# kernrj/cuda-sdr

Measured on AMD Instinct MI355X. Metric: Msamples/sec through FIR→QuadAmDemod chain at 1/2/4/8 MI355X; % HBM roofline, higher is better.
Workload: dtype f32

## Files before the change

### cuda-sdr_amd/csrc/kernels/fir.hip

```cpp
#include "kcommon.h"
#include "fir_launch.h"

#include <gsdr/gsdr.h>
#include <gsdr/gsdr_amd.h>

#include <atomic>
#include <cmath>
#include <type_traits>
#include <utility>

namespace gsdr_amd {

enum InKind : int { kInF32 = 0, kInCF32 = 1, kInI8IQ = 2 };

constexpr int kR = 8;
constexpr int kRowBytes = 80;
constexpr int kThreads = 256;
constexpr int kWaves = kThreads / kWave;
constexpr int kWaveOutputs = kWave * kR;
constexpr int kFlushGroups = 8;

struct FirArgs {
  const void* in;
  const float* taps;
// ... 637 lines not shown

struct MixSpec {
  bool on = false;
  uint64_t phase0 = 0, step = 0;
};

template <int... Q>
void (*decFFTable(std::integer_sequence<int, Q...>, int qm))(FirArgs) {
  static void (*const kTable[])(FirArgs) = {firDecFFKernel<Q + 1>...};
  return kTable[qm - 1];
}
inline void (*decFFKernel(int qm))(FirArgs) { return decFFTable(std::make_integer_sequence<int, kDecMaxQ>{}, qm); }

template <int MODE, int INK, int EPI>
hipError_t launchFir(const void* in, const float* taps, size_t tapCount, size_t decimation, void* out,
                     size_t nOut, int32_t device, hipStream_t stream, MixSpec mix = MixSpec{}, float fmGain = 0.0f) {
  if (nOut == 0) return hipSuccess;
  if (in == nullptr || taps == nullptr || out == nullptr || tapCount == 0) return hipErrorInvalidValue;
  if (tapCount > 0x7fffffff || decimation > 0x7fffffff) return hipErrorInvalidValue;
  DevicePush push(device);
  if (!push.ok) return hipErrorInvalidDevice;

  if constexpr (MODE == kFirFC && (INK == kInI8IQ || INK == kInCF32) && EPI != kEpiPair && EPI != kEpiFm) {
    const bool smallCf = kFftSmallToMfma && INK == kInCF32 && !mix.on && decimation >= 2 &&
                         (uint64_t)nOut * decimation < kFftMinCf32Samples &&
                         (kernelPolicy() & (GSDR_POLICY_NO_MFMA | GSDR_POLICY_PREFER_FFT)) == 0 &&
                         firCfMfmaEligible(tapCount, decimation, in);
    if (!smallCf && (kernelPolicy() & (GSDR_POLICY_NO_FFT | GSDR_POLICY_NO_MFMA)) == 0 &&
        firFftEligible(tapCount, decimation, in, INK == kInI8IQ, mix.on))
      return launchFirFft(in, INK == kInI8IQ, taps, tapCount, decimation, out, nOut, EPI, stream,
                          FftMix{mix.on, mix.phase0, mix.step});
  }
  if constexpr (MODE == kFirCC && INK == kInCF32 && (EPI == kEpiComplex || EPI == kEpiAm)) {
    if (!mix.on && (kernelPolicy() & (GSDR_POLICY_NO_FFT | GSDR_POLICY_NO_MFMA)) == 0 &&
        firFftEligible(tapCount, decimation, in, false, false))
      return launchFirFft(in, false, taps, tapCount, decimation, out, nOut, EPI, stream, FftMix{}, true);
  }
  if constexpr (MODE == kFirFC && INK == kInI8IQ && EPI != kEpiPair && EPI != kEpiFm) if (!mix.on) {
    if ((kernelPolicy() & GSDR_POLICY_NO_MFMA) == 0 && firI8MfmaEligible(tapCount, decimation, in))
      return launchFirI8Mfma(static_cast<const int8_t*>(in), taps, tapCount, out, nOut, EPI, stream);
    if ((kernelPolicy() & GSDR_POLICY_NO_MFMA) == 0 && firI8DecMfmaEligible(tapCount, decimation, in))
      return launchFirI8DecMfma(static_cast<const int8_t*>(in), taps, tapCount, decimation, out, nOut, EPI, stream);
  }
  if constexpr (MODE == kFirFC && INK == kInCF32 && EPI != kEpiPair && EPI != kEpiFm) if (!mix.on) {
    if ((kernelPolicy() & GSDR_POLICY_NO_MFMA) == 0 && firCfMfmaEligible(tapCount, decimation, in))
      return launchFirCfMfma(static_cast<const float*>(in), taps, tapCount, decimation, out, nOut, EPI, stream);
  }

  const FirPlanShape s = planFirShape(tapCount, decimation);
  FirArgs a{};
  a.in = in;
// ... 256 lines not shown

hipError_t gsdrInt8MixFirFCAmDemod(size_t decimation, const float* taps, size_t tapCount, const int8_t* inputIq,
                                   double phase0, double radiansPerSample, float* output, size_t outputCount,
                                   int32_t device, hipStream_t stream) {
  return launchFir<kFirFC, kInI8IQ, kEpiAm>(inputIq, taps, tapCount, decimation, output, outputCount, device, stream,
                                            mixSpec(phase0, radiansPerSample));
}

hipError_t gsdrFirCCAmDemod(size_t decimation, const hipFloatComplex* taps, size_t tapCount,
                            const hipFloatComplex* input, float* output, size_t outputCount, int32_t device,
                            hipStream_t stream) {
  return launchFir<kFirCC, kInCF32, kEpiAm>(input, reinterpret_cast<const float*>(taps), tapCount, decimation,
                                            output, outputCount, device, stream);
}

}
```

### cuda-sdr_amd/csrc/kernels/fir_fft.hip

```cpp
#include "kcommon.h"
#include "fir_launch.h"

#include <gsdr/gsdr.h>
#include <gsdr/gsdr_amd.h>

#include <atomic>
#include <cmath>


namespace gsdr_amd {
namespace fftfir {

__device__ unsigned long long gDirectBlocks;

#ifndef GSDR_FFT_STAMPS
#define GSDR_FFT_STAMPS 0
#endif
#ifndef GSDR_FFT_EXP
#define GSDR_FFT_EXP 0
#endif
#if GSDR_FFT_STAMPS
constexpr int kStampWaves = 256 * 8;
__device__ unsigned long long gFftStamps[kStampWaves * 4];
#endif
// ... 11 lines not shown
  const float* taps;
  void* out;
  int64_t nOut;
  int64_t inBytes;
  int64_t nBlocks;
  int64_t inRows;
  int32_t T;
  int32_t Q;
  int32_t V;
  float inScale;
  float guardRatio;
  uint64_t mixPhase0;
  uint64_t mixStep;
  int32_t outAligned;
  int32_t complexTaps;
};

__device__ __forceinline__ f2 tapAt(const Args& a, int j) {
  return a.complexTaps ? reinterpret_cast<const f2*>(a.taps)[j] : f2{a.taps[j], 0.0f};
}

__device__ __forceinline__ f2 turnExp(uint64_t frac) {
  double sn, cs;
  sincospi((double)(int64_t)frac * 1.0842021724855044e-19, &sn, &cs);
  return f2{(float)cs, (float)sn};
}
__device__ __forceinline__ f2 turnExpF(uint64_t frac) {
  const int32_t hi = (int32_t)(frac >> 40) << 8 >> 8;
  float sh, ch;
  sincospif((float)hi * 1.1920928955078125e-7f, &sh, &ch);
// ... 254 lines not shown
template <int D>
constexpr int kRowUnits = D / 2 + ((GSDR_FFT_PADROWS && D == 4) ? 1 : 0);
template <int D>
__device__ __forceinline__ int rowSwizzle(int row) {
  return D == 8 ? (row >> 2) & 3 : 0;
}

template <int D>
constexpr int scratchComplex(int input) {
  return input == kCf32 ? (128 * kRowUnits<D> > 2 * kXch ? 128 * kRowUnits<D> : 2 * kXch)
                        : ((1024 * D + 16) / 8 > 2 * kXch ? (1024 * D + 16 + 7) / 8 : 2 * kXch);
}

constexpr int kMixT = 8 * 64;

template <int D, int IN, bool MIX = false>
constexpr size_t ldsBytes() {
  return (size_t)(D * 8 * 64 + kTw + kWaves * scratchComplex<D>(IN) + (MIX ? kMixT : 0)) * sizeof(f2);
}

template <int D, int IN, int NW = kWaves, bool MIX = false>
__device__ void buildTables(const Args& a, f2* twAll, const Lds& L, int w, int l, f2* mixT = nullptr) {
  if constexpr (MIX) {
    for (int n = threadIdx.x; n < kMixT; n += NW * kWave) {
      const int lane = (n >> 1) & 63, j = 2 * (n >> 7) + (n & 1);
      mixT[n] = turnExp((uint64_t)((lane + 64 * j) * D) * a.mixStep);
    }
  }
  for (int n = threadIdx.x; n < kTw; n += NW * kWave) {
    const int stage = n >> 9, kp = (n >> 7) & 3, lane = (n >> 1) & 63, r = 2 * kp + (n & 1) + 1;
    const int lo = lane & 7, hi = lane >> 3;
    int e;
    switch (stage) {
      case 0: e = lane * r; break;
// ... 286 lines not shown
    }
  }
}

#ifndef GSDR_FFT_XCD
#define GSDR_FFT_XCD 1
#endif
__device__ __forceinline__ int xcdGroup(int i, int n) {
  if (!GSDR_FFT_XCD || (n & 7) != 0) return i;
  return (i & 7) * (n >> 3) + (i >> 3);
}
#ifndef GSDR_FFT_XCD_D
#define GSDR_FFT_XCD_D 0
#endif

template <int D, int IN, int EPI, bool MIX = false>
__global__ void __launch_bounds__(kThreads) firFftKernel(Args a) {
  extern __shared__ __attribute__((aligned(16))) f2 lds[];
  const int w = __builtin_amdgcn_readfirstlane(threadIdx.x >> 6), l = threadIdx.x & 63;
  f2* twAll = lds + D * 8 * 64;
  f2* mixT = twAll + kTw + kWaves * scratchComplex<D>(IN);
  Lds L;
  L.g = reinterpret_cast<f4*>(lds);
  L.tw = reinterpret_cast<const f4*>(twAll) + l;
  L.scratch = twAll + kTw + w * scratchComplex<D>(IN);
  buildTables<D, IN, kWaves, MIX>(a, twAll, L, w, l, mixT);
#if GSDR_FFT_STAMPS
  const unsigned long long st0 = __builtin_amdgcn_s_memtime(), rt0 = __builtin_amdgcn_s_memrealtime();
#endif

  const int64_t stride = (int64_t)gridDim.x * kWaves;
  const int grp = GSDR_FFT_XCD_D ? xcdGroup((int)blockIdx.x, (int)gridDim.x) : (int)blockIdx.x;
  for (int64_t b = (int64_t)grp * kWaves + w; b < a.nBlocks; b += stride) {
    Rows<D, IN> R;
    loadRows<D>(a, b, R, L.scratch, l);
    f2 t[8];
    if constexpr (MIX) {
      loadMixT(t, reinterpret_cast<const f4*>(mixT), l);
      if constexpr (IN == kCf32) {
#pragma unroll
        for (int j = 0; j < 8; ++j)
#pragma unroll
          for (int p = 0; p < D; ++p) R.v[j][p] = cmul(R.v[j][p], t[j]);
      }
    }
    if (!(GSDR_FFT_EXP & 8) && blockNeedsDirect<D, IN>(a, R, b, l)) {
      if (l == 0) atomicAdd(&gDirectBlocks, 1ull);
      directBlock<D, IN, EPI, MIX>(a, b, l);
      continue;
    }
    __builtin_amdgcn_s_setprio(2);
    convolveBlock<D, IN, EPI, MIX>(a, R, b, L, l, t);
    __builtin_amdgcn_s_setprio(0);
  }
#if GSDR_FFT_STAMPS
  const unsigned long long st1 = __builtin_amdgcn_s_memtime(), rt1 = __builtin_amdgcn_s_memrealtime();
  const int slot = (int)blockIdx.x * kWaves + w;
  if (l == 0 && slot < kStampWaves) {
    unsigned long long* s = gFftStamps + 4 * slot;
    s[0] = st0;
    s[1] = rt0;
    s[2] = st1;
    s[3] = rt1;
  }
#endif
}

constexpr int kPfWaves = 4;

template <int D>
struct PrefetchCf {
  f4 u[8][D / 2];
};

template <int D>
__device__ __forceinline__ void issueBlockLoads(const Args& a, int64_t b, PrefetchCf<D>& P, int l) {
  const int64_t off = b < a.nBlocks ? b * (int64_t)a.V * D * 8 : 0;
  const auto rs = blockRsrc((const char*)a.in + off, b < a.nBlocks ? a.inBytes - off : 0);
#pragma unroll
  for (int j = 0; j < 8; ++j)
// ... 242 lines not shown
}

}

namespace {

std::atomic<float> gFftGuard{8.0f};

int cuCount() {
  int dev = 0, n = 0;
  if (hipGetDevice(&dev) != hipSuccess || hipDeviceGetAttribute(&n, hipDeviceAttributeMultiprocessorCount, dev) != hipSuccess || n <= 0)
    return 256;
  return n;
}

template <int D, int IN, int EPI, bool MIX>
hipError_t launchD(fftfir::Args a, hipStream_t stream) {
  using namespace fftfir;
  auto kernel = firFftKernel<D, IN, EPI, MIX>;
  const size_t lds = ldsBytes<D, IN, MIX>();
  const hipError_t e = hipFuncSetAttribute((const void*)kernel, hipFuncAttributeMaxDynamicSharedMemorySize, (int)lds);
  if (e != hipSuccess) return e;
  const int64_t maxGroups = cuCount();
  int64_t groups = (a.nBlocks + kWaves - 1) / kWaves;
  if (groups > maxGroups) groups = maxGroups;

  hipLaunchKernelGGL(kernel, dim3((unsigned)groups), dim3(kThreads), lds, stream, a);
  return hipGetLastError();
}

template <int EPI>
hipError_t launchD1(fftfir::Args a, hipStream_t stream) {
  using namespace fftfir;
  auto kernel = firFftD1PfKernel<EPI>;
  const size_t lds = (size_t)(8 * 8 * 64 + kTw + kPfWaves * scratchComplex<8>(kCf32) + kTwD1) * sizeof(f2);
  const hipError_t e = hipFuncSetAttribute((const void*)kernel, hipFuncAttributeMaxDynamicSharedMemorySize, (int)lds);
  if (e != hipSuccess) return e;
  const int64_t maxGroups = cuCount();
  int64_t groups = (a.nBlocks + kPfWaves - 1) / kPfWaves;
  if (groups > maxGroups) groups = maxGroups;
  hipLaunchKernelGGL(kernel, dim3((unsigned)groups), dim3(kPfWaves * kWave), lds, stream, a);
  return hipGetLastError();
}
// ... 25 lines not shown
    if (mixed) return false;
    const size_t Q = (tapCount + 7) / 8;
    return !int8Iq && tapCount >= 256 && Q <= (size_t)fftfir::kM - 64 && ((uintptr_t)in & 15) == 0;
  }
  if (!(D == 2 || D == 4 || D == 6 || D == 8 || D == 10)) return false;
  const size_t Q = (tapCount + D - 1) / D;
  if (tapCount < 256 || Q > (size_t)fftfir::kM - 63) return false;
  const uintptr_t p = (uintptr_t)in;
  if (int8Iq)
    return (p & 3) == 0 && (mixed || (kernelPolicy() & GSDR_POLICY_PREFER_FFT) != 0 ||
                            (!firI8MfmaEligible(tapCount, decimation, in) && !firI8DecMfmaEligible(tapCount, decimation, in)));
  return (p & 15) == 0;
}

hipError_t launchFirFft(const void* in, bool int8Iq, const float* taps, size_t tapCount, size_t decimation,
                        void* out, size_t nOut, int epi, hipStream_t stream, FftMix mix, bool complexTaps) {
  using namespace fftfir;
  if (nOut == 0) return hipSuccess;
  if (complexTaps && (int8Iq || mix.on)) return hipErrorInvalidValue;
  const size_t D = decimation < 1 ? 1 : decimation;
  if (D == 1) {
    if (int8Iq || mix.on) return hipErrorInvalidValue;
    Args a{};
    a.in = in;
    a.taps = taps;
    a.out = out;
    a.nOut = (int64_t)nOut;
    a.T = (int32_t)tapCount;
    a.Q = (int32_t)((tapCount + 7) / 8);
    a.V = kM - a.Q;
    a.inBytes = (int64_t)(nOut - 1 + tapCount) * 8;
// ... 7 lines not shown
  }
  Args a{};
  a.in = in;
  a.taps = taps;
  a.out = out;
  a.nOut = (int64_t)nOut;
  a.T = (int32_t)tapCount;
  a.Q = (int32_t)((tapCount + D - 1) / D);
  a.V = kM - a.Q + 1;
  a.inBytes = (int64_t)((nOut - 1) * D + tapCount) * (int8Iq ? 2 : 8);
  a.nBlocks = ((int64_t)nOut + a.V - 1) / a.V;
  a.inRows = (int64_t)(((nOut - 1) * D + tapCount) / D);
  a.inScale = int8Iq ? 1.0f / 127.0f : 1.0f;
  a.guardRatio = gFftGuard.load(std::memory_order_relaxed);
  a.complexTaps = complexTaps ? 1 : 0;
  const bool am = epi == kEpiAm;
  if (mix.on) {
    a.mixPhase0 = mix.phase0;
    a.mixStep = mix.step;
    if (int8Iq) return am ? launchFft<kI8, kAm, true>(a, D, stream) : launchFft<kI8, kComplex, true>(a, D, stream);
    return am ? launchFft<kCf32, kAm, true>(a, D, stream) : launchFft<kCf32, kComplex, true>(a, D, stream);
  }
  if (int8Iq) return am ? launchFft<kI8, kAm>(a, D, stream) : launchFft<kI8, kComplex>(a, D, stream);
  return am ? launchFft<kCf32, kAm>(a, D, stream) : launchFft<kCf32, kComplex>(a, D, stream);
}

}

extern "C" {
void gsdrAmdSetFftGuard(float ratio) { gsdr_amd::gFftGuard.store(ratio, std::memory_order_relaxed); }
float gsdrAmdGetFftGuard(void) { return gsdr_amd::gFftGuard.load(std::memory_order_relaxed); }

hipError_t gsdrAmdFftDirectBlocks(int32_t device, uint64_t* count, int reset) {
  int prev = 0;
  hipError_t e = hipGetDevice(&prev);
  if (e != hipSuccess) return e;
  if ((e = hipSetDevice(device)) != hipSuccess) return e;
  unsigned long long v = 0;
  e = hipDeviceSynchronize();
// ... 11 lines not shown
```

### cuda-sdr_amd/csrc/kernels/fir_launch.h

```cpp
#pragma once

#include <stddef.h>

namespace gsdr_amd {

enum FirMode : int { kFirFF = 0, kFirFC = 1, kFirCC = 2, kFirCF = 3 };
enum FirEpilogue : int { kEpiComplex = 0, kEpiPair = 1, kEpiAm = 2, kEpiFm = 3 };

struct FirPlanShape {
  size_t decimation;
  size_t deff;
  size_t gtot;
  size_t gmax;
  int waveOutputSlices;
  size_t regionRows;
  size_t ldsBytes;
  size_t tileOutputs;
};

FirPlanShape planFirShape(size_t tapCount, size_t decimation);

}

#include <hip/hip_runtime_api.h>
// ... 11 lines not shown

bool firI8DecMfmaEligible(size_t tapCount, size_t decimation, const void* in);
hipError_t launchFirI8DecMfma(const int8_t* iq, const float* taps, size_t tapCount, size_t decimation, void* out,
                              size_t nOut, int epi, hipStream_t stream);
hipError_t launchFirI8DecMfmaAudio(const int8_t* iq, const float* taps, size_t tapCount, size_t decimation,
                                   float* amOut, size_t nOut, const float* amHist, size_t amH, const float* aTaps,
                                   size_t aT, size_t aD, float* aOut, size_t aN, hipStream_t stream);

struct FftMix {
  bool on = false;
  uint64_t phase0 = 0, step = 0;
};
bool firFftEligible(size_t tapCount, size_t decimation, const void* in, bool int8Iq, bool mixed = false);
hipError_t launchFirFft(const void* in, bool int8Iq, const float* taps, size_t tapCount, size_t decimation,
                        void* out, size_t nOut, int epi, hipStream_t stream, FftMix mix = FftMix{},
                        bool complexTaps = false);

uint32_t kernelPolicy();

}
```

### cuda-sdr_amd/csrc/runtime/filters.cpp

```cpp
#include "filters.h"

#include <cstring>

#include <gsdr/conversion.h>
#include <gsdr/gsdr.h>
#include <gsdr/gsdr_amd.h>

#include <algorithm>
#include <cmath>

namespace gsdr_rt {

namespace {

Result<std::vector<ImmutableRef<IBufferCopier>>> deviceOutputCopiers(IFactories* f, ICudaCommandQueue* q) noexcept {
  try {
    Ref<IBufferCopier> d2d;
    UNWRAP_OR_FWD_RESULT(d2d, f->getCudaBufferCopierFactory()->createBufferCopier(q, hipMemcpyDeviceToDevice));
    std::vector<ImmutableRef<IBufferCopier>> v;
    v.emplace_back(d2d.get().get());
    return {.status = Status_Success, .value = std::move(v)};
  }
  IF_CATCH_RETURN_RESULT;
}
// ... 50 lines not shown
      mElementType(elementType),
      mAllocator(allocator),
      mH2D(h2d),
      mDecimation(std::max<size_t>(1, decimation)),
      mQueue(queue),
      mInElem(inputElementSize(elementType)),
      mOutElem((tapType == SampleType_Float && elementType == SampleType_Float) ? sizeof(float)
                                                                                : 2 * sizeof(float)) {}

Status Fir::setTaps(const float* taps, size_t tapCount) noexcept {
  GS_REQUIRE_OR_RET_STATUS(taps != nullptr || tapCount == 0, "taps must be non-null when tapCount > 0");
  const size_t bytes = tapCount * (mTapType == SampleType_FloatComplex ? 2 * sizeof(float) : sizeof(float));
  if (mTaps == nullptr || mTaps->capacity() < bytes) UNWRAP_OR_FWD_STATUS(mTaps, mAllocator->allocate(bytes));
  if (bytes > 0) FWD_IF_ERR(mH2D->copy(mTaps->data(), taps, bytes));
  mTapCount = tapCount;
  return Status_Success;
}

size_t Fir::availableInputs() const noexcept {
  if (!inputPortsInitialized()) return 0;
  Result<const IBuffer> in = getPortInputBuffer(0);
  if (in.status != Status_Success) return 0;
  return in.value->range()->used() / mInElem;
}

size_t Fir::availableOutputs() const noexcept {
  const size_t n = availableInputs();
  if (mTapCount == 0 || n < mTapCount) return 0;
  return (n - (mTapCount - 1)) / mDecimation;
}

size_t Fir::getOutputDataSize(size_t port) noexcept {
// ... 8 lines not shown

Status Fir::readOutput(IBuffer** portOutputBuffers, size_t portCount) noexcept {
  GS_REQUIRE_OR_RET_STATUS(portCount != 0 && portOutputBuffers != nullptr && portOutputBuffers[0] != nullptr,
                           "Must have one output port");
  IBuffer* out = portOutputBuffers[0];
  Ref<IBuffer> in;
  UNWRAP_OR_FWD_STATUS(in, getPortInputBuffer(0));
  const size_t n = std::min(availableOutputs(), out->range()->remaining() / mOutElem);
  if (n == 0) return Status_Success;

  const int32_t dev = mQueue->cudaDevice();
  hipStream_t s = mQueue->cudaStream();
  const void* x = in->readPtr();
  void* y = out->writePtr();
  hipError_t e;
  if (mElementType == SampleType_Int8Complex) {
    e = gsdrInt8FirFC(mDecimation, mTaps->as<float>(), mTapCount, static_cast<const int8_t*>(x),
                      static_cast<hipFloatComplex*>(y), n, dev, s);
  } else if (mTapType == SampleType_Float && mElementType == SampleType_Float) {
    e = gsdrFirFF(mDecimation, mTaps->as<float>(), mTapCount, static_cast<const float*>(x), static_cast<float*>(y), n,
                  dev, s);
  } else if (mTapType == SampleType_Float) {
    e = gsdrFirFC(mDecimation, mTaps->as<float>(), mTapCount, static_cast<const hipFloatComplex*>(x),
                  static_cast<hipFloatComplex*>(y), n, dev, s);
  } else if (mElementType == SampleType_FloatComplex) {
    e = gsdrFirCC(mDecimation, mTaps->as<hipFloatComplex>(), mTapCount, static_cast<const hipFloatComplex*>(x),
                  static_cast<hipFloatComplex*>(y), n, dev, s);
  } else {
    e = gsdrFirCF(mDecimation, mTaps->as<hipFloatComplex>(), mTapCount, static_cast<const float*>(x),
                  static_cast<hipFloatComplex*>(y), n, dev, s);
  }
  SAFE_HIP_OR_RET_STATUS(e);
  FWD_IF_ERR(out->range()->increaseEndOffset(n * mOutElem));
  return consumeInputBytesAndMoveUsedToStart(0, n * mDecimation * mInElem);
}

Status Fir::readOutputAm(IBuffer* out) noexcept {
  GS_REQUIRE_OR_RET_STATUS(out != nullptr && canFuseAm(), "Fir::readOutputAm needs real taps and an output");
  Ref<IBuffer> in;
  UNWRAP_OR_FWD_STATUS(in, getPortInputBuffer(0));
  const size_t n = std::min(availableOutputs(), out->range()->remaining() / sizeof(float));
  if (n == 0) return Status_Success;
  const int32_t dev = mQueue->cudaDevice();
  hipStream_t s = mQueue->cudaStream();
  hipError_t e;
  if (mElementType == SampleType_Int8Complex)
    e = gsdrInt8FirFCAmDemod(mDecimation, mTaps->as<float>(), mTapCount, in->readPtr<int8_t>(), out->writePtr<float>(),
                             n, dev, s);
  else
    e = gsdrFirFCAmDemod(mDecimation, mTaps->as<float>(), mTapCount, in->readPtr<hipFloatComplex>(),
                         out->writePtr<float>(), n, dev, s);
  SAFE_HIP_OR_RET_STATUS(e);
  FWD_IF_ERR(out->range()->increaseEndOffset(n * sizeof(float)));
  return consumeInputBytesAndMoveUsedToStart(0, n * mDecimation * mInElem);
}

Result<Filter> QuadAmDemod::create(ICudaCommandQueue* queue, IFactories* factories) noexcept {
  NON_NULL_PARAM_OR_RET(queue);
  Ref<IRelocatableResizableBufferFactory> windows;
  Ref<IMemSet> memSet;
  UNWRAP_OR_FWD_RESULT(windows, factories->createRelocatableCudaBufferFactory(queue, 32, false));
// ... 392 lines not shown
```

### cuda-sdr_amd/csrc/runtime/filters.h

```cpp
#pragma once

#include "waiter.h"

#include <gpusdrpipeline/Factories.h>
#include <gpusdrpipeline/abi/base_filters.h>
#include <gpusdrpipeline/abi/errors.h>

#include "graph_state.h"

namespace gsdr_rt {

constexpr size_t kDevicePreferredBytes = size_t{256} << 20;

size_t inputElementSize(SampleType t) noexcept;

class Fir final : public BaseFilter, public IGraphStepState {
 public:
  hipStream_t graphStream() const noexcept final { return mQueue->cudaStream(); }
  bool graphState(uint64_t& h) const noexcept final {
    foldWindowState(h);
    h = (h ^ reinterpret_cast<uintptr_t>(mTaps.get() ? mTaps->data() : nullptr)) * 0x100000001B3ull + mTapCount;
    return true;
  }
  bool saveStepState(GraphNodeState& out) const noexcept final { return saveSinkWindows(*this, out); }
  Status restoreStepState(const GraphNodeState& in) noexcept final { return restoreSinkWindows(*this, in); }
  static Result<Filter> create(SampleType tapType, SampleType elementType, size_t decimation, const float* taps,
                               size_t tapCount, ICudaCommandQueue* queue, IFactories* factories) noexcept;

  size_t getOutputDataSize(size_t port) noexcept final;
  size_t getOutputSizeAlignment(size_t port) noexcept final;
  Status readOutput(IBuffer** portOutputBuffers, size_t numPorts) noexcept final;
  size_t preferredInputBufferSize(size_t port) noexcept final { return kDevicePreferredBytes; }

  size_t decimation() const noexcept { return mDecimation; }
  size_t tapCount() const noexcept { return mTapCount; }

// ... 8 lines not shown
 private:
  Fir(SampleType tapType, SampleType elementType, size_t decimation, ICudaCommandQueue* queue, IAllocator* allocator,
      IBufferCopier* h2d, IRelocatableResizableBufferFactory* windows, IBufferSliceFactory* slices, IMemSet* memSet,
      std::vector<ImmutableRef<IBufferCopier>>&& outputCopiers) noexcept;
  Status setTaps(const float* taps, size_t tapCount) noexcept;
  size_t availableInputs() const noexcept;
  size_t availableOutputs() const noexcept;

  const SampleType mTapType;
  const SampleType mElementType;
  ConstRef<IAllocator> mAllocator;
  ConstRef<IBufferCopier> mH2D;
  const size_t mDecimation;
  Ref<IMemory> mTaps;
  size_t mTapCount = 0;
  ConstRef<ICudaCommandQueue> mQueue;
  const size_t mInElem;
  const size_t mOutElem;

  REF_COUNTED(Fir);
};

class QuadAmDemod final : public BaseFilter, public IGraphStepState {
 public:
  hipStream_t graphStream() const noexcept final { return mQueue->cudaStream(); }
  bool graphState(uint64_t& h) const noexcept final {
    foldWindowState(h);
    return true;
  }
  bool saveStepState(GraphNodeState& out) const noexcept final { return saveSinkWindows(*this, out); }
  Status restoreStepState(const GraphNodeState& in) noexcept final { return restoreSinkWindows(*this, in); }
  static Result<Filter> create(ICudaCommandQueue* queue, IFactories* factories) noexcept;
  size_t getOutputDataSize(size_t port) noexcept final;
  size_t getOutputSizeAlignment(size_t port) noexcept final;
  Status readOutput(IBuffer** portOutputBuffers, size_t numPorts) noexcept final;
// ... 175 lines not shown
```

### cuda-sdr_amd/gpusdr/ops.py

```python
from __future__ import annotations

import ctypes

import torch

from ._native import HipError, check, lib


def _stream(t: torch.Tensor):
    return torch.cuda.current_stream(t.device).cuda_stream


def _dev(t: torch.Tensor) -> int:
    return t.device.index if t.device.index is not None else torch.cuda.current_device()


def _require(t: torch.Tensor, dtype, name: str):
    if not t.is_cuda:
        raise ValueError(f"{name} must be a device tensor")
    if t.dtype != dtype:
        raise ValueError(f"{name} must be {dtype}, got {t.dtype}")
    if not t.is_contiguous():
        raise ValueError(f"{name} must be contiguous")

# ... 83 lines not shown
    if out.numel() < num_outputs:
        raise ValueError("out too small")
    fn = getattr(lib(), _FIR_ENTRY[key])
    args = (d, taps.data_ptr(), T, x.data_ptr(), out.data_ptr(), int(num_outputs), _dev(x), _stream(x))
    name = fn.__name__
    keep = (taps, x, out)

    def launch():
        if num_outputs > 0:
            code = fn(*args)
            if code != 0:
                raise HipError(f"{name} failed with hipError_t {code} ({len(keep)} bound tensors)")
    return launch


def fir_am_i8_carry(taps: torch.Tensor, iq: torch.Tensor, decimation: int, num_outputs: int,
                    out: torch.Tensor, carry: torch.Tensor) -> torch.Tensor:
    _require(taps, torch.float32, "taps")
    _require(iq, torch.int8, "iq")
    _require(out, torch.float32, "out")
    _require(carry, torch.int8, "carry")
    d = max(1, int(decimation))
    T = taps.numel()
    if num_outputs > 0 and (num_outputs - 1) * d + T > iq.numel() // 2:
        raise ValueError("input too short for the requested outputs")
    if out.numel() < num_outputs or carry.numel() < 2 * max(0, T - d):
        raise ValueError("out or carry too small")
    check(lib().gsdrInt8FirFCAmDemodCarry(d, taps.data_ptr(), T, iq.data_ptr(), out.data_ptr(), num_outputs,
                                          carry.data_ptr(), _dev(iq), _stream(iq)), "gsdrInt8FirFCAmDemodCarry")
    return out
# ... 112 lines not shown
def synth_wideband_cf32(seed: int, f1: float, f2: float, first: int, n: int,
                        out: torch.Tensor | None = None, device="cuda") -> torch.Tensor:
    if out is None:
        out = torch.empty(n, dtype=torch.complex64, device=device)
    check(lib().gsdrSynthWidebandCf32(seed, f1, f2, first, out.data_ptr(), n, _dev(out), _stream(out)),
          "gsdrSynthWidebandCf32")
    return out


POLICY_NO_MFMA = 1
POLICY_CF_BF16 = 2
POLICY_NO_WS = 4
POLICY_NO_FFT = 8
POLICY_PREFER_FFT = 16
POLICY_I8_WS8 = 64


def kernel_policy() -> int:
    L = lib()
    L.gsdrAmdGetKernelPolicy.restype = ctypes.c_uint32
    return int(L.gsdrAmdGetKernelPolicy())


def set_kernel_policy(flags: int) -> int:
    L = lib()
    L.gsdrAmdGetKernelPolicy.restype = ctypes.c_uint32
    L.gsdrAmdSetKernelPolicy.argtypes = [ctypes.c_uint32]
    prev = L.gsdrAmdGetKernelPolicy()
    L.gsdrAmdSetKernelPolicy(flags)
    return prev
# ... 77 lines not shown
```

### include/gsdr/gsdr_amd.h

```cpp
#ifndef GSDR_GSDR_AMD_H
#define GSDR_GSDR_AMD_H

#include <gsdr/gsdr.h>

#ifdef __cplusplus
extern "C" {
#endif

GSDR_API hipError_t gsdrInt8FirFC(size_t decimation, const float* taps, size_t tapCount, const int8_t* inputIq,
                                  hipFloatComplex* output, size_t outputCount, int32_t device, hipStream_t stream);
GSDR_API hipError_t gsdrInt8FirFCAmDemod(size_t decimation, const float* taps, size_t tapCount,
                                         const int8_t* inputIq, float* output, size_t outputCount, int32_t device,
                                         hipStream_t stream);
GSDR_API hipError_t gsdrFirFCAmDemod(size_t decimation, const float* taps, size_t tapCount,
                                     const hipFloatComplex* input, float* output, size_t outputCount, int32_t device,
                                     hipStream_t stream);
GSDR_API hipError_t gsdrFirCCAmDemod(size_t decimation, const hipFloatComplex* taps, size_t tapCount,
                                     const hipFloatComplex* input, float* output, size_t outputCount, int32_t device,
                                     hipStream_t stream);

GSDR_API hipError_t gsdrInt8FirFCAmDemodFirFF(size_t decimation, const float* taps, size_t tapCount,
                                              const int8_t* inputIq, size_t rfCount, float* amWindow,
                                              size_t amHistory, int storeAm, size_t audioDecimation,
                                              const float* audioTaps, size_t audioTapCount, float* audioOut,
// ... 22 lines not shown
                                        hipStream_t stream);
GSDR_API hipError_t gsdrInt8MixFirFCFmDemod(size_t decimation, const float* taps, size_t tapCount,
                                            const int8_t* inputIq, double phase0, double radiansPerSample, float gain,
                                            float* output, size_t outputCount, int32_t device, hipStream_t stream);
GSDR_API hipError_t gsdrFmDemod(size_t rfSampleRate, float tunedFrequency, float channelFrequency,
                                float channelFmDeviation, size_t rfLowPassDecimation, size_t firstSampleOffset,
                                const float* taps, size_t tapCount, const hipFloatComplex* input, float* output,
                                size_t outputCount, int32_t device, hipStream_t stream);

#define GSDR_POLICY_NO_MFMA 1u
#define GSDR_POLICY_CF_BF16 2u
#define GSDR_POLICY_NO_WS 4u
#define GSDR_POLICY_NO_FFT 8u
#define GSDR_POLICY_PREFER_FFT 16u
#define GSDR_POLICY_I8_WS8 64u
GSDR_API void gsdrAmdSetKernelPolicy(uint32_t flags);
GSDR_API const char* gsdrAmdFirKernelClass(int int8Iq, size_t tapCount, size_t decimation, const void* input);
GSDR_API uint32_t gsdrAmdGetKernelPolicy(void);
GSDR_API void gsdrAmdSetFftGuard(float ratio);
GSDR_API float gsdrAmdGetFftGuard(void);
GSDR_API hipError_t gsdrAmdFftDirectBlocks(int32_t device, uint64_t* count, int reset);
GSDR_API void gsdrAmdSetWsSpinLimit(int32_t microseconds);
GSDR_API int32_t gsdrAmdGetWsSpinLimit(void);
GSDR_API hipError_t gsdrAmdWsAborts(int32_t device, uint64_t* count, int reset);
GSDR_API uint32_t gsdrAmdWsTakeAborts(int32_t device);
GSDR_API uint32_t gsdrAmdWsAbortsPending(int32_t device);
GSDR_API const char* gsdrAmdBuildId(void);
GSDR_API const char* gsdrAmdBuildCompiler(void);
GSDR_API hipError_t gsdrAmdHbmProbe(const void* input, void* output, size_t bytes, int32_t mode, int32_t device,
                                    hipStream_t stream);
GSDR_API hipError_t gsdrAmdPoisonLds(uint32_t pattern, int32_t device, hipStream_t stream);
GSDR_API hipError_t gsdrAmdCopyKernel(void* dst, const void* src, size_t bytes, hipStream_t stream);

GSDR_API hipError_t gsdrSynthIqInt8(uint64_t seed, double sampleRate, double amToneHz, double carrierHz,
                                    uint64_t firstSample, int8_t* outputIq, size_t numSamples, int32_t device,
// ... 62 lines not shown
```

Baseline: 545,100.

## Add FIR plan with precomputed FFT tables and narrower FFT blocks for small grids

```diff
diff --git a/cuda-sdr_amd/csrc/kernels/fir.hip b/cuda-sdr_amd/csrc/kernels/fir.hip
--- a/cuda-sdr_amd/csrc/kernels/fir.hip
+++ b/cuda-sdr_amd/csrc/kernels/fir.hip
@@ -675,7 +675,8 @@
 
 template <int MODE, int INK, int EPI>
 hipError_t launchFir(const void* in, const float* taps, size_t tapCount, size_t decimation, void* out,
-                     size_t nOut, int32_t device, hipStream_t stream, MixSpec mix = MixSpec{}, float fmGain = 0.0f) {
+                     size_t nOut, int32_t device, hipStream_t stream, MixSpec mix = MixSpec{}, float fmGain = 0.0f,
+                     const void* fftTables = nullptr) {
   if (nOut == 0) return hipSuccess;
   if (in == nullptr || taps == nullptr || out == nullptr || tapCount == 0) return hipErrorInvalidValue;
   if (tapCount > 0x7fffffff || decimation > 0x7fffffff) return hipErrorInvalidValue;
@@ -690,12 +691,12 @@
     if (!smallCf && (kernelPolicy() & (GSDR_POLICY_NO_FFT | GSDR_POLICY_NO_MFMA)) == 0 &&
         firFftEligible(tapCount, decimation, in, INK == kInI8IQ, mix.on))
       return launchFirFft(in, INK == kInI8IQ, taps, tapCount, decimation, out, nOut, EPI, stream,
-                          FftMix{mix.on, mix.phase0, mix.step});
+                          FftMix{mix.on, mix.phase0, mix.step}, false, fftTables);
   }
   if constexpr (MODE == kFirCC && INK == kInCF32 && (EPI == kEpiComplex || EPI == kEpiAm)) {
     if (!mix.on && (kernelPolicy() & (GSDR_POLICY_NO_FFT | GSDR_POLICY_NO_MFMA)) == 0 &&
         firFftEligible(tapCount, decimation, in, false, false))
-      return launchFirFft(in, false, taps, tapCount, decimation, out, nOut, EPI, stream, FftMix{}, true);
+      return launchFirFft(in, false, taps, tapCount, decimation, out, nOut, EPI, stream, FftMix{}, true, fftTables);
   }
   if constexpr (MODE == kFirFC && INK == kInI8IQ && EPI != kEpiPair && EPI != kEpiFm) if (!mix.on) {
     if ((kernelPolicy() & GSDR_POLICY_NO_MFMA) == 0 && firI8MfmaEligible(tapCount, decimation, in))
@@ -982,4 +983,49 @@
                                             output, outputCount, device, stream);
 }
 
-}
+hipError_t gsdrAmdFirPlanCreate(int32_t device, hipStream_t stream, const void* taps, size_t tapCount,
+                                size_t decimation, int32_t int8Iq, int32_t complexTaps, gsdrAmdFirPlan* planOut) {
+  if (planOut == nullptr) return hipErrorInvalidValue;
+  *planOut = nullptr;
+  DevicePush push(device);
+  if (!push.ok) return hipErrorInvalidDevice;
+  FirFftPlan* p = nullptr;
+  const hipError_t e = firFftPlanCreate(device, stream, static_cast<const float*>(taps), tapCount, decimation,
+                                        int8Iq != 0, complexTaps != 0, &p);
+  if (e == hipSuccess) *planOut = reinterpret_cast<gsdrAmdFirPlan>(p);
+  return e;
+}
+
+void gsdrAmdFirPlanDestroy(gsdrAmdFirPlan plan) {
+  FirFftPlan* p = reinterpret_cast<FirFftPlan*>(plan);
+  if (p == nullptr) return;
+  DevicePush push(p->device);
+  firFftPlanDestroy(p);
+}
+
+const void* gsdrAmdFirPlanTables(gsdrAmdFirPlan plan) {
+  return plan != nullptr ? reinterpret_cast<const FirFftPlan*>(plan)->tables : nullptr;
+}
+
+hipError_t gsdrAmdFirPlanLaunch(gsdrAmdFirPlan plan, int32_t amDemod, const void* input, void* output,
+                                size_t outputCount, hipStream_t stream) {
+  const FirFftPlan* p = reinterpret_cast<const FirFftPlan*>(plan);
+  if (p == nullptr) return hipErrorInvalidValue;
+  const size_t D = p->decimation, T = p->tapCount;
+  if (p->int8Iq)
+    return amDemod ? launchFir<kFirFC, kInI8IQ, kEpiAm>(input, p->taps, T, D, output, outputCount, p->device, stream,
+                                                        MixSpec{}, 0.0f, p->tables)
+                   : launchFir<kFirFC, kInI8IQ, kEpiComplex>(input, p->taps, T, D, output, outputCount, p->device,
+                                                             stream, MixSpec{}, 0.0f, p->tables);
+  if (p->complexTaps)
+    return amDemod ? launchFir<kFirCC, kInCF32, kEpiAm>(input, p->taps, T, D, output, outputCount, p->device, stream,
+                                                        MixSpec{}, 0.0f, p->tables)
+                   : launchFir<kFirCC, kInCF32, kEpiComplex>(input, p->taps, T, D, output, outputCount, p->device,
+                                                             stream, MixSpec{}, 0.0f, p->tables);
+  return amDemod ? launchFir<kFirFC, kInCF32, kEpiAm>(input, p->taps, T, D, output, outputCount, p->device, stream,
+                                                      MixSpec{}, 0.0f, p->tables)
+                 : launchFir<kFirFC, kInCF32, kEpiComplex>(input, p->taps, T, D, output, outputCount, p->device,
+                                                           stream, MixSpec{}, 0.0f, p->tables);
+}
+
+}
diff --git a/cuda-sdr_amd/csrc/kernels/fir_fft.hip b/cuda-sdr_amd/csrc/kernels/fir_fft.hip
--- a/cuda-sdr_amd/csrc/kernels/fir_fft.hip
+++ b/cuda-sdr_amd/csrc/kernels/fir_fft.hip
@@ -6,6 +6,7 @@
 
 #include <atomic>
 #include <cmath>
+#include <new>
 
 
 namespace gsdr_amd {
@@ -49,6 +50,7 @@
   uint64_t mixStep;
   int32_t outAligned;
   int32_t complexTaps;
+  const void* tables;
 };
 
 __device__ __forceinline__ f2 tapAt(const Args& a, int j) {
@@ -333,10 +335,12 @@
 
 constexpr int kMixT = 8 * 64;
 
-template <int D, int IN, bool MIX = false>
+template <int D, int IN, bool MIX = false, int NW = kWaves>
 constexpr size_t ldsBytes() {
-  return (size_t)(D * 8 * 64 + kTw + kWaves * scratchComplex<D>(IN) + (MIX ? kMixT : 0)) * sizeof(f2);
-}
+  return (size_t)(D * 8 * 64 + kTw + NW * scratchComplex<D>(IN) + (MIX ? kMixT : 0)) * sizeof(f2);
+}
+template <int D>
+constexpr int kTableUnits = (D * 8 * 64 + kTw) / 2;
 
 template <int D, int IN, int NW = kWaves, bool MIX = false>
 __device__ void buildTables(const Args& a, f2* twAll, const Lds& L, int w, int l, f2* mixT = nullptr) {
@@ -653,24 +657,31 @@
 #define GSDR_FFT_XCD_D 0
 #endif
 
-template <int D, int IN, int EPI, bool MIX = false>
-__global__ void __launch_bounds__(kThreads) firFftKernel(Args a) {
+template <int D, int IN, int EPI, bool MIX = false, int NW = kWaves>
+__global__ void __launch_bounds__(NW * kWave) firFftKernel(Args a) {
   extern __shared__ __attribute__((aligned(16))) f2 lds[];
   const int w = __builtin_amdgcn_readfirstlane(threadIdx.x >> 6), l = threadIdx.x & 63;
   f2* twAll = lds + D * 8 * 64;
-  f2* mixT = twAll + kTw + kWaves * scratchComplex<D>(IN);
+  f2* mixT = twAll + kTw + NW * scratchComplex<D>(IN);
   Lds L;
   L.g = reinterpret_cast<f4*>(lds);
   L.tw = reinterpret_cast<const f4*>(twAll) + l;
   L.scratch = twAll + kTw + w * scratchComplex<D>(IN);
-  buildTables<D, IN, kWaves, MIX>(a, twAll, L, w, l, mixT);
+  if (!MIX && a.tables != nullptr) {
+    const f4* src = reinterpret_cast<const f4*>(a.tables);
+    f4* dst = reinterpret_cast<f4*>(lds);
+    for (int n = threadIdx.x; n < kTableUnits<D>; n += NW * kWave) dst[n] = src[n];
+    __syncthreads();
+  } else {
+    buildTables<D, IN, NW, MIX>(a, twAll, L, w, l, mixT);
+  }
 #if GSDR_FFT_STAMPS
   const unsigned long long st0 = __builtin_amdgcn_s_memtime(), rt0 = __builtin_amdgcn_s_memrealtime();
 #endif
 
-  const int64_t stride = (int64_t)gridDim.x * kWaves;
+  const int64_t stride = (int64_t)gridDim.x * NW;
   const int grp = GSDR_FFT_XCD_D ? xcdGroup((int)blockIdx.x, (int)gridDim.x) : (int)blockIdx.x;
-  for (int64_t b = (int64_t)grp * kWaves + w; b < a.nBlocks; b += stride) {
+  for (int64_t b = (int64_t)grp * NW + w; b < a.nBlocks; b += stride) {
     Rows<D, IN> R;
     loadRows<D>(a, b, R, L.scratch, l);
     f2 t[8];
@@ -694,7 +705,7 @@
   }
 #if GSDR_FFT_STAMPS
   const unsigned long long st1 = __builtin_amdgcn_s_memtime(), rt1 = __builtin_amdgcn_s_memrealtime();
-  const int slot = (int)blockIdx.x * kWaves + w;
+  const int slot = (int)blockIdx.x * NW + w;
   if (l == 0 && slot < kStampWaves) {
     unsigned long long* s = gFftStamps + 4 * slot;
     s[0] = st0;
@@ -703,6 +714,20 @@
     s[3] = rt1;
   }
 #endif
+}
+
+template <int D>
+__global__ void __launch_bounds__(kThreads) firFftTablesKernel(Args a, f4* image) {
+  extern __shared__ __attribute__((aligned(16))) f2 lds[];
+  const int w = __builtin_amdgcn_readfirstlane(threadIdx.x >> 6), l = threadIdx.x & 63;
+  f2* twAll = lds + D * 8 * 64;
+  Lds L;
+  L.g = reinterpret_cast<f4*>(lds);
+  L.tw = reinterpret_cast<const f4*>(twAll) + l;
+  L.scratch = twAll + kTw + w * scratchComplex<D>(kCf32);
+  buildTables<D, kCf32, kWaves, false>(a, twAll, L, w, l);
+  const f4* src = reinterpret_cast<const f4*>(lds);
+  for (int n = threadIdx.x; n < kTableUnits<D>; n += kThreads) image[n] = src[n];
 }
 
 constexpr int kPfWaves = 4;
@@ -975,19 +1000,31 @@
   return n;
 }
 
+template <int D, int IN, int EPI, bool MIX, int NW>
+hipError_t launchNW(fftfir::Args a, int64_t maxGroups, hipStream_t stream) {
+  using namespace fftfir;
+  auto kernel = firFftKernel<D, IN, EPI, MIX, NW>;
+  const size_t lds = ldsBytes<D, IN, MIX, NW>();
+  const hipError_t e = hipFuncSetAttribute((const void*)kernel, hipFuncAttributeMaxDynamicSharedMemorySize, (int)lds);
+  if (e != hipSuccess) return e;
+  int64_t groups = (a.nBlocks + NW - 1) / NW;
+  if (groups > maxGroups) groups = maxGroups;
+
+  hipLaunchKernelGGL(kernel, dim3((unsigned)groups), dim3(NW * kWave), lds, stream, a);
+  return hipGetLastError();
+}
+
 template <int D, int IN, int EPI, bool MIX>
 hipError_t launchD(fftfir::Args a, hipStream_t stream) {
   using namespace fftfir;
-  auto kernel = firFftKernel<D, IN, EPI, MIX>;
-  const size_t lds = ldsBytes<D, IN, MIX>();
-  const hipError_t e = hipFuncSetAttribute((const void*)kernel, hipFuncAttributeMaxDynamicSharedMemorySize, (int)lds);
-  if (e != hipSuccess) return e;
-  const int64_t maxGroups = cuCount();
-  int64_t groups = (a.nBlocks + kWaves - 1) / kWaves;
-  if (groups > maxGroups) groups = maxGroups;
-
-  hipLaunchKernelGGL(kernel, dim3((unsigned)groups), dim3(kThreads), lds, stream, a);
-  return hipGetLastError();
+  const int64_t cus = cuCount();
+  if constexpr (!MIX) {
+    if (a.nBlocks < cus * kWaves && (kernelPolicy() & GSDR_POLICY_FFT_GRID8) == 0) {
+      if (a.nBlocks <= cus * 2) return launchNW<D, IN, EPI, MIX, 2>(a, cus, stream);
+      if (a.nBlocks <= cus * 4) return launchNW<D, IN, EPI, MIX, 4>(a, cus, stream);
+    }
+  }
+  return launchNW<D, IN, EPI, MIX, kWaves>(a, cus, stream);
 }
 
 template <int EPI>
@@ -1043,7 +1080,8 @@
 }
 
 hipError_t launchFirFft(const void* in, bool int8Iq, const float* taps, size_t tapCount, size_t decimation,
-                        void* out, size_t nOut, int epi, hipStream_t stream, FftMix mix, bool complexTaps) {
+                        void* out, size_t nOut, int epi, hipStream_t stream, FftMix mix, bool complexTaps,
+                        const void* tables) {
   using namespace fftfir;
   if (nOut == 0) return hipSuccess;
   if (complexTaps && (int8Iq || mix.on)) return hipErrorInvalidValue;
@@ -1081,6 +1119,7 @@
   a.inScale = int8Iq ? 1.0f / 127.0f : 1.0f;
   a.guardRatio = gFftGuard.load(std::memory_order_relaxed);
   a.complexTaps = complexTaps ? 1 : 0;
+  a.tables = mix.on ? nullptr : tables;
   const bool am = epi == kEpiAm;
   if (mix.on) {
     a.mixPhase0 = mix.phase0;
@@ -1090,6 +1129,72 @@
   }
   if (int8Iq) return am ? launchFft<kI8, kAm>(a, D, stream) : launchFft<kI8, kComplex>(a, D, stream);
   return am ? launchFft<kCf32, kAm>(a, D, stream) : launchFft<kCf32, kComplex>(a, D, stream);
+}
+
+namespace {
+template <int D>
+hipError_t launchTables(fftfir::Args a, void* image, hipStream_t stream) {
+  using namespace fftfir;
+  auto kernel = firFftTablesKernel<D>;
+  const size_t lds = ldsBytes<D, kCf32>();
+  const hipError_t e = hipFuncSetAttribute((const void*)kernel, hipFuncAttributeMaxDynamicSharedMemorySize, (int)lds);
+  if (e != hipSuccess) return e;
+  hipLaunchKernelGGL(kernel, dim3(1), dim3(kThreads), lds, stream, a, reinterpret_cast<f4*>(image));
+  return hipGetLastError();
+}
+}
+
+hipError_t firFftPlanCreate(int32_t device, hipStream_t stream, const float* taps, size_t tapCount, size_t decimation,
+                            bool int8Iq, bool complexTaps, FirFftPlan** planOut) {
+  using namespace fftfir;
+  if (planOut == nullptr) return hipErrorInvalidValue;
+  *planOut = nullptr;
+  if (taps == nullptr || tapCount == 0 || tapCount > 0x7fffffff || decimation > 0x7fffffff || (int8Iq && complexTaps))
+    return hipErrorInvalidValue;
+  const size_t D = decimation < 1 ? 1 : decimation;
+  FirFftPlan* p = new (std::nothrow) FirFftPlan;
+  if (p == nullptr) return hipErrorOutOfMemory;
+  p->device = device;
+  p->tapCount = tapCount;
+  p->decimation = D;
+  p->int8Iq = int8Iq;
+  p->complexTaps = complexTaps;
+  const size_t tapBytes = tapCount * (complexTaps ? 8 : 4);
+  hipError_t e = hipMalloc(reinterpret_cast<void**>(&p->taps), tapBytes);
+  if (e == hipSuccess) e = hipMemcpyAsync(p->taps, taps, tapBytes, hipMemcpyDeviceToDevice, stream);
+  const size_t Q = (tapCount + D - 1) / D;
+  const bool shape = (D == 2 || D == 4 || D == 6 || D == 8 || D == 10) && tapCount >= 256 && Q <= (size_t)kM - 63;
+  if (e == hipSuccess && shape) {
+    e = hipMalloc(&p->tables, (D * 8 * 64 + kTw) * sizeof(f2));
+    if (e == hipSuccess) {
+      Args a{};
+      a.taps = p->taps;
+      a.T = (int32_t)tapCount;
+      a.Q = (int32_t)Q;
+      a.inScale = int8Iq ? 1.0f / 127.0f : 1.0f;
+      a.complexTaps = complexTaps ? 1 : 0;
+      switch (D) {
+        case 2: e = launchTables<2>(a, p->tables, stream); break;
+        case 4: e = launchTables<4>(a, p->tables, stream); break;
+        case 6: e = launchTables<6>(a, p->tables, stream); break;
+        case 8: e = launchTables<8>(a, p->tables, stream); break;
+        default: e = launchTables<10>(a, p->tables, stream); break;
+      }
+    }
+  }
+  if (e != hipSuccess) {
+    firFftPlanDestroy(p);
+    return e;
+  }
+  *planOut = p;
+  return hipSuccess;
+}
+
+void firFftPlanDestroy(FirFftPlan* p) {
+  if (p == nullptr) return;
+  if (p->tables != nullptr) (void)hipFree(p->tables);
+  if (p->taps != nullptr) (void)hipFree(p->taps);
+  delete p;
 }
 
 }
diff --git a/cuda-sdr_amd/csrc/kernels/fir_launch.h b/cuda-sdr_amd/csrc/kernels/fir_launch.h
--- a/cuda-sdr_amd/csrc/kernels/fir_launch.h
+++ b/cuda-sdr_amd/csrc/kernels/fir_launch.h
@@ -49,7 +49,18 @@
 bool firFftEligible(size_t tapCount, size_t decimation, const void* in, bool int8Iq, bool mixed = false);
 hipError_t launchFirFft(const void* in, bool int8Iq, const float* taps, size_t tapCount, size_t decimation,
                         void* out, size_t nOut, int epi, hipStream_t stream, FftMix mix = FftMix{},
-                        bool complexTaps = false);
+                        bool complexTaps = false, const void* tables = nullptr);
+
+struct FirFftPlan {
+  int32_t device = 0;
+  float* taps = nullptr;
+  void* tables = nullptr;
+  size_t tapCount = 0, decimation = 1;
+  bool int8Iq = false, complexTaps = false;
+};
+hipError_t firFftPlanCreate(int32_t device, hipStream_t stream, const float* taps, size_t tapCount, size_t decimation,
+                            bool int8Iq, bool complexTaps, FirFftPlan** planOut);
+void firFftPlanDestroy(FirFftPlan* plan);
 
 uint32_t kernelPolicy();
 
diff --git a/cuda-sdr_amd/csrc/runtime/filters.cpp b/cuda-sdr_amd/csrc/runtime/filters.cpp
--- a/cuda-sdr_amd/csrc/runtime/filters.cpp
+++ b/cuda-sdr_amd/csrc/runtime/filters.cpp
@@ -88,8 +88,20 @@
   if (mTaps == nullptr || mTaps->capacity() < bytes) UNWRAP_OR_FWD_STATUS(mTaps, mAllocator->allocate(bytes));
   if (bytes > 0) FWD_IF_ERR(mH2D->copy(mTaps->data(), taps, bytes));
   mTapCount = tapCount;
+  if (mPlan != nullptr) {
+    gsdrAmdFirPlanDestroy(mPlan);
+    mPlan = nullptr;
+  }
+  const bool planned = tapCount > 0 && (mElementType == SampleType_Int8Complex ||
+                                        (mElementType == SampleType_FloatComplex && isFloatOrComplex(mTapType)));
+  if (planned)
+    SAFE_HIP_OR_RET_STATUS(gsdrAmdFirPlanCreate(mQueue->cudaDevice(), mQueue->cudaStream(), mTaps->data(), tapCount,
+                                                mDecimation, mElementType == SampleType_Int8Complex,
+                                                mTapType == SampleType_FloatComplex, &mPlan));
   return Status_Success;
 }
+
+Fir::~Fir() { gsdrAmdFirPlanDestroy(mPlan); }
 
 size_t Fir::availableInputs() const noexcept {
   if (!inputPortsInitialized()) return 0;
@@ -128,7 +140,9 @@
   const void* x = in->readPtr();
   void* y = out->writePtr();
   hipError_t e;
-  if (mElementType == SampleType_Int8Complex) {
+  if (mPlan != nullptr) {
+    e = gsdrAmdFirPlanLaunch(mPlan, 0, x, y, n, s);
+  } else if (mElementType == SampleType_Int8Complex) {
     e = gsdrInt8FirFC(mDecimation, mTaps->as<float>(), mTapCount, static_cast<const int8_t*>(x),
                       static_cast<hipFloatComplex*>(y), n, dev, s);
   } else if (mTapType == SampleType_Float && mElementType == SampleType_Float) {
@@ -158,7 +172,9 @@
   const int32_t dev = mQueue->cudaDevice();
   hipStream_t s = mQueue->cudaStream();
   hipError_t e;
-  if (mElementType == SampleType_Int8Complex)
+  if (mPlan != nullptr)
+    e = gsdrAmdFirPlanLaunch(mPlan, 1, in->readPtr(), out->writePtr(), n, s);
+  else if (mElementType == SampleType_Int8Complex)
     e = gsdrInt8FirFCAmDemod(mDecimation, mTaps->as<float>(), mTapCount, in->readPtr<int8_t>(), out->writePtr<float>(),
                              n, dev, s);
   else
diff --git a/cuda-sdr_amd/csrc/runtime/filters.h b/cuda-sdr_amd/csrc/runtime/filters.h
--- a/cuda-sdr_amd/csrc/runtime/filters.h
+++ b/cuda-sdr_amd/csrc/runtime/filters.h
@@ -6,6 +6,8 @@
 #include <gpusdrpipeline/abi/base_filters.h>
 #include <gpusdrpipeline/abi/errors.h>
 
+#include <gsdr/gsdr_amd.h>
+
 #include "graph_state.h"
 
 namespace gsdr_rt {
@@ -20,6 +22,7 @@
   bool graphState(uint64_t& h) const noexcept final {
     foldWindowState(h);
     h = (h ^ reinterpret_cast<uintptr_t>(mTaps.get() ? mTaps->data() : nullptr)) * 0x100000001B3ull + mTapCount;
+    h = (h ^ reinterpret_cast<uintptr_t>(gsdrAmdFirPlanTables(mPlan))) * 0x100000001B3ull;
     return true;
   }
   bool saveStepState(GraphNodeState& out) const noexcept final { return saveSinkWindows(*this, out); }
@@ -58,11 +61,13 @@
   const size_t mDecimation;
   Ref<IMemory> mTaps;
   size_t mTapCount = 0;
+  gsdrAmdFirPlan mPlan = nullptr;
   ConstRef<ICudaCommandQueue> mQueue;
   const size_t mInElem;
   const size_t mOutElem;
 
-  REF_COUNTED(Fir);
+  ~Fir() final;
+  REF_COUNTED_NO_DESTRUCTOR(Fir);
 };
 
 class QuadAmDemod final : public BaseFilter, public IGraphStepState {
diff --git a/cuda-sdr_amd/gpusdr/ops.py b/cuda-sdr_amd/gpusdr/ops.py
--- a/cuda-sdr_amd/gpusdr/ops.py
+++ b/cuda-sdr_amd/gpusdr/ops.py
@@ -121,6 +121,68 @@
     return launch
 
 
+class FirPlan:
+
+    def __init__(self, taps: torch.Tensor, decimation: int, int8_iq: bool = False):
+        self.taps_complex = taps.dtype == torch.complex64
+        _require(taps, torch.complex64 if self.taps_complex else torch.float32, "taps")
+        if int8_iq and self.taps_complex:
+            raise ValueError("int8 IQ input needs real taps")
+        self.decimation, self.int8_iq, self.tap_count = max(1, int(decimation)), bool(int8_iq), taps.numel()
+        self.device = _dev(taps)
+        self._h = ctypes.c_void_p()
+        L = lib()
+        L.gsdrAmdFirPlanCreate.argtypes = [ctypes.c_int32, ctypes.c_void_p, ctypes.c_void_p, ctypes.c_size_t,
+                                           ctypes.c_size_t, ctypes.c_int32, ctypes.c_int32,
+                                           ctypes.POINTER(ctypes.c_void_p)]
+        L.gsdrAmdFirPlanLaunch.argtypes = [ctypes.c_void_p, ctypes.c_int32, ctypes.c_void_p, ctypes.c_void_p,
+                                           ctypes.c_size_t, ctypes.c_void_p]
+        L.gsdrAmdFirPlanDestroy.argtypes = [ctypes.c_void_p]
+        L.gsdrAmdFirPlanDestroy.restype = None
+        L.gsdrAmdFirPlanTables.argtypes = [ctypes.c_void_p]
+        L.gsdrAmdFirPlanTables.restype = ctypes.c_void_p
+        check(L.gsdrAmdFirPlanCreate(self.device, _stream(taps), taps.data_ptr(), self.tap_count, self.decimation,
+                                     1 if int8_iq else 0, 1 if self.taps_complex else 0, ctypes.byref(self._h)),
+              "gsdrAmdFirPlanCreate")
+
+    @property
+    def tables(self) -> int:
+        return int(lib().gsdrAmdFirPlanTables(self._h) or 0) if self._h else 0
+
+    def __call__(self, x: torch.Tensor, num_outputs: int | None = None, out: torch.Tensor | None = None,
+                 am: bool = False) -> torch.Tensor:
+        if not self._h:
+            raise ValueError("plan destroyed")
+        _require(x, torch.int8 if self.int8_iq else torch.complex64, "x")
+        n_in = x.numel() // 2 if self.int8_iq else x.numel()
+        if num_outputs is None:
+            num_outputs = fir_output_count(n_in, self.tap_count, self.decimation)
+        if num_outputs > 0 and (num_outputs - 1) * self.decimation + self.tap_count > n_in:
+            raise ValueError("input too short for the requested outputs")
+        out_dtype = torch.float32 if am else torch.complex64
+        if out is None:
+            out = torch.empty(num_outputs, dtype=out_dtype, device=x.device)
+        else:
+            _require(out, out_dtype, "out")
+            if out.numel() < num_outputs:
+                raise ValueError("out too small")
+        if num_outputs > 0:
+            check(lib().gsdrAmdFirPlanLaunch(self._h, 1 if am else 0, x.data_ptr(), out.data_ptr(), num_outputs,
+                                             _stream(x)), "gsdrAmdFirPlanLaunch")
+        return out
+
+    def destroy(self) -> None:
+        if self._h:
+            lib().gsdrAmdFirPlanDestroy(self._h)
+            self._h = ctypes.c_void_p()
+
+    def __del__(self):
+        try:
+            self.destroy()
+        except Exception:
+            pass
+
+
 def fir_am_i8_carry(taps: torch.Tensor, iq: torch.Tensor, decimation: int, num_outputs: int,
                     out: torch.Tensor, carry: torch.Tensor) -> torch.Tensor:
     _require(taps, torch.float32, "taps")
@@ -263,6 +325,7 @@
 POLICY_NO_FFT = 8
 POLICY_PREFER_FFT = 16
 POLICY_I8_WS8 = 64
+POLICY_FFT_GRID8 = 128
 
 
 def kernel_policy() -> int:
diff --git a/include/gsdr/gsdr_amd.h b/include/gsdr/gsdr_amd.h
--- a/include/gsdr/gsdr_amd.h
+++ b/include/gsdr/gsdr_amd.h
@@ -60,11 +60,20 @@
 #define GSDR_POLICY_NO_FFT 8u
 #define GSDR_POLICY_PREFER_FFT 16u
 #define GSDR_POLICY_I8_WS8 64u
+#define GSDR_POLICY_FFT_GRID8 128u
 GSDR_API void gsdrAmdSetKernelPolicy(uint32_t flags);
 GSDR_API const char* gsdrAmdFirKernelClass(int int8Iq, size_t tapCount, size_t decimation, const void* input);
 GSDR_API uint32_t gsdrAmdGetKernelPolicy(void);
 GSDR_API void gsdrAmdSetFftGuard(float ratio);
 GSDR_API float gsdrAmdGetFftGuard(void);
+typedef struct gsdrAmdFirPlanImpl* gsdrAmdFirPlan;
+GSDR_API hipError_t gsdrAmdFirPlanCreate(int32_t device, hipStream_t stream, const void* taps, size_t tapCount,
+                                         size_t decimation, int32_t int8Iq, int32_t complexTaps,
+                                         gsdrAmdFirPlan* planOut);
+GSDR_API void gsdrAmdFirPlanDestroy(gsdrAmdFirPlan plan);
+GSDR_API hipError_t gsdrAmdFirPlanLaunch(gsdrAmdFirPlan plan, int32_t amDemod, const void* input, void* output,
+                                         size_t outputCount, hipStream_t stream);
+GSDR_API const void* gsdrAmdFirPlanTables(gsdrAmdFirPlan plan);
 GSDR_API hipError_t gsdrAmdFftDirectBlocks(int32_t device, uint64_t* count, int reset);
 GSDR_API void gsdrAmdSetWsSpinLimit(int32_t microseconds);
 GSDR_API int32_t gsdrAmdGetWsSpinLimit(void);
```

Result: no change. 544,700 (-0.1%).
